# facebookresearch/GPU-DPF

Measured on AMD Instinct MI355X. Metric: DPFs/sec, higher is better.
Workload: dtype int32; 1 GPU; model=dpf-pir, entries=1048576, entry_size=16, prf=AES128, batch_per_gpu=512, global_batch=512, parallelism=dp1-replicated

## Files before the change

### csrc/hip/prf_device.h

```cpp
#pragma once
#include "hip_util.h"

namespace gpudpf_hip {

__device__ __forceinline__ uint4 add128(uint4 a, uint4 b) {
  u64 alo = ((u64)a.y << 32) | a.x, ahi = ((u64)a.w << 32) | a.z;
  u64 blo = ((u64)b.y << 32) | b.x, bhi = ((u64)b.w << 32) | b.z;
  u64 lo = alo + blo;
  u64 hi = ahi + bhi + (lo < alo ? 1u : 0u);
  return make_uint4((u32)lo, (u32)(lo >> 32), (u32)hi, (u32)(hi >> 32));
}

__device__ __forceinline__ u32 rotl(u32 v, int s) {
  return (v << s) | (v >> (32 - s));
}
__device__ __forceinline__ u32 rotr8(u32 v) { return (v >> 8) | (v << 24); }

__device__ __forceinline__ uint4 key_root(const int* key) {
  const int* rp = key + kKeyRootInt;
  return make_uint4((u32)rp[0], (u32)rp[1], (u32)rp[2], (u32)rp[3]);
}

__device__ __forceinline__ uint4 prf_dummy_full(uint4 seed, u32 pos) {
  unsigned __int128 s =
      ((unsigned __int128)(((u64)seed.w << 32) | seed.z) << 64) |
      (((u64)seed.y << 32) | seed.x);
  unsigned __int128 m = (unsigned __int128)(pos + 4242u);
  unsigned __int128 r = s * m + m;
  u64 lo = (u64)r, hi = (u64)(r >> 64);
  return make_uint4((u32)lo, (u32)(lo >> 32), (u32)hi, (u32)(hi >> 32));
}

template <int N>
__device__ __forceinline__ void stream_init(u32 (&x)[16][N], int pos_w,
                                            const u32 (&init)[16]) {
#pragma unroll
  for (int w = 0; w < 16; ++w)
#pragma unroll
    for (int i = 0; i < N; ++i) x[w][i] = init[w] + (w == pos_w ? i : 0);
}

template <int N>
__device__ __forceinline__ uint4 stream_out(const u32 (&x)[16][N], int i,
                                            int lo, uint4 seed) {
  return make_uint4(x[lo][i] + seed.x, x[lo - 1][i] + seed.y,
                    x[lo - 2][i] + seed.z, x[lo - 3][i] + seed.w);
}

template <int PART = 4, int N>
__device__ __forceinline__ void salsa_qr(u32 (&x)[16][N], int a, int b, int c,
                                         int d) {
  auto step = [&](int t, int p, int q, int s) {
#pragma unroll
    for (int i = 0; i < N; ++i) x[t][i] ^= rotl(x[p][i] + x[q][i], s);
  };
  step(b, a, d, 7);
  if constexpr (PART > 1) step(c, b, a, 9);
  if constexpr (PART > 2) step(d, c, b, 13);
  if constexpr (PART > 3) step(a, d, c, 18);
}

template <bool LOW, int N>
__device__ __forceinline__ void salsa12(uint4 seed, u32 pos, u32 (&x)[16][N]) {
  stream_init(x, 9, {0x65787061u, seed.w, seed.z, seed.y, seed.x, 0x6e642033u,
                     0, 0, 0, pos, 0x322d6279u, 0, 0, 0, 0, 0x7465206bu});
#pragma unroll
  for (int r = 0; r < (LOW ? 5 : 6); ++r) {
    salsa_qr(x, 0, 4, 8, 12);
    salsa_qr(x, 5, 9, 13, 1);
    salsa_qr(x, 10, 14, 2, 6);
    salsa_qr(x, 15, 3, 7, 11);
    salsa_qr(x, 0, 1, 2, 3);
    salsa_qr(x, 5, 6, 7, 4);
    salsa_qr(x, 10, 11, 8, 9);
    salsa_qr(x, 15, 12, 13, 14);
  }
  if constexpr (LOW) {
    salsa_qr<1>(x, 0, 4, 8, 12);
    salsa_qr(x, 5, 9, 13, 1);
    salsa_qr<3>(x, 10, 14, 2, 6);
    salsa_qr<2>(x, 15, 3, 7, 11);
    salsa_qr<3>(x, 5, 6, 7, 4);
  }
}

__device__ __forceinline__ uint4 salsa12_core(uint4 seed, u32 pos) {
  u32 x[16][1];
  salsa12<false>(seed, pos, x);
  return stream_out(x, 0, 4, seed);
}

__device__ __forceinline__ void salsa12_pair_core(uint4 seed, uint4& r0,
                                                  uint4& r1) {
  u32 x[16][2];
  salsa12<false>(seed, 0, x);
  r0 = stream_out(x, 0, 4, seed);
  r1 = stream_out(x, 1, 4, seed);
}

__device__ __forceinline__ void salsa12_pair_low_core(uint4 seed, u32& lo0,
                                                      u32& lo1) {
  u32 x[16][2];
  salsa12<true>(seed, 0, x);
  lo0 = x[4][0] + seed.x;
  lo1 = x[4][1] + seed.x;
}

template <int PART = 8, int N>
__device__ __forceinline__ void chacha_qr(u32 (&x)[16][N], int a, int b, int c,
                                          int d) {
  static_assert(PART >= 6 && PART <= 8, "only the tail is ever pruned");
  auto add = [&](int t, int s) {
#pragma unroll
    for (int i = 0; i < N; ++i) x[t][i] += x[s][i];
  };
  auto xor_rotl = [&](int t, int s, int r) {
#pragma unroll
    for (int i = 0; i < N; ++i) x[t][i] ^= x[s][i];
#pragma unroll
    for (int i = 0; i < N; ++i) x[t][i] = rotl(x[t][i], r);
  };
  add(a, b);  xor_rotl(d, a, 16);
  add(c, d);  xor_rotl(b, c, 12);
  add(a, b);  xor_rotl(d, a, 8);
  if constexpr (PART > 6) add(c, d);
  if constexpr (PART > 7) xor_rotl(b, c, 7);
}

template <bool LOW, int N>
__device__ __forceinline__ void chacha12(uint4 seed, u32 pos,
                                         u32 (&x)[16][N]) {
  stream_init(x, 13, {0x65787061u, 0x6e642033u, 0x322d6279u, 0x7465206bu,
                      seed.w, seed.z, seed.y, seed.x, 0, 0, 0, 0, 0, pos, 0, 0});
#pragma unroll
  for (int r = 0; r < (LOW ? 5 : 6); ++r) {
    chacha_qr(x, 0, 4, 8, 12);
    chacha_qr(x, 1, 5, 9, 13);
    chacha_qr(x, 2, 6, 10, 14);
    chacha_qr(x, 3, 7, 11, 15);
    chacha_qr(x, 0, 5, 10, 15);
    chacha_qr(x, 1, 6, 11, 12);
    chacha_qr(x, 2, 7, 8, 13);
    chacha_qr(x, 3, 4, 9, 14);
  }
  if constexpr (LOW) {
    chacha_qr<7>(x, 0, 4, 8, 12);
    chacha_qr<6>(x, 1, 5, 9, 13);
    chacha_qr(x, 2, 6, 10, 14);
    chacha_qr(x, 3, 7, 11, 15);
    chacha_qr(x, 2, 7, 8, 13);
  }
}

__device__ __forceinline__ uint4 chacha12_core(uint4 seed, u32 pos) {
  u32 x[16][1];
  chacha12<false>(seed, pos, x);
  return stream_out(x, 0, 7, seed);
}

__device__ __forceinline__ void chacha12_pair_core(uint4 seed, uint4& r0,
                                                   uint4& r1) {
  u32 x[16][2];
  chacha12<false>(seed, 0, x);
  r0 = stream_out(x, 0, 7, seed);
  r1 = stream_out(x, 1, 7, seed);
}

__device__ __forceinline__ void chacha12_pair_low_core(uint4 seed, u32& lo0,
                                                       u32& lo1) {
  u32 x[16][2];
  chacha12<true>(seed, 0, x);
  lo0 = x[7][0] + seed.x;
  lo1 = x[7][1] + seed.x;
}

constexpr int AES_COPIES = 32;
constexpr int AES_REP = AES_COPIES * 2;
constexpr int AES_LDS_WORDS = 256 * AES_REP;
constexpr u32 AES_TE2_BYTES = AES_COPIES * 4;

__host__ __device__ constexpr int aes_lds_u32(int prf) {
  return prf == PRF_AES128 ? AES_LDS_WORDS : 0;
}

__device__ __forceinline__ u32 xor3(u32 a, u32 b, u32 c) {
  return __builtin_amdgcn_bitop3_b32(a, b, c, 0x96);
}

template <int PA, int PB, int BA = 2, int BB = 2>
__device__ __forceinline__ u32 aes_sb_pair(u32 ta, u32 tb) {
  static_assert(PA != PB, "the two bytes land in different places");
  constexpr u32 sel = (0x0c0c0c0cu & ~(0xffu << (8 * PA)) &
                       ~(0xffu << (8 * PB))) |
                      ((4u + BA) << (8 * PA)) | ((u32)BB << (8 * PB));
  return __builtin_amdgcn_perm(ta, tb, sel);
}

__device__ __forceinline__ u32 bswap_rol8(u32 x) {
  return __builtin_amdgcn_perm(0u, x, 0x01020300u);
}

struct AesLds {
  u32 lane4;
  static __device__ __forceinline__ AesLds lane() {
    return AesLds{((u32)threadIdx.x & (u32)(AES_COPIES - 1)) << 2};
  }
  typedef __attribute__((address_space(3))) const u32 lds_u32;
  static __device__ __forceinline__ u32 ld(u32 byte_addr) {
    return *reinterpret_cast<lds_u32*>(byte_addr);
  }
  static __device__ __forceinline__ u32 ld_te2(u32 byte_addr) {
    return reinterpret_cast<lds_u32*>(byte_addr)[AES_TE2_BYTES / 4];
  }
  template <int K>
  __device__ __forceinline__ u32 addr_b(u32 w) const {
    return __builtin_amdgcn_perm(w, lane4, 0x0c0c0000u | ((4u + K) << 8));
  }
  template <int K>
  __device__ __forceinline__ u32 te0_b(u32 w) const { return ld(addr_b<K>(w)); }
  template <int K>
  __device__ __forceinline__ u32 te2_b(u32 w) const {
    return ld_te2(addr_b<K>(w));
  }
  template <int K>
  __device__ __forceinline__ u32 addr_kb(u32 q) const {
    return addr_b<(K + 1) & 3>(q);
  }
  template <int K>
  __device__ __forceinline__ u32 te0_kb(u32 q) const { return ld(addr_kb<K>(q)); }
  template <int K>
  __device__ __forceinline__ u32 te2_kb(u32 q) const {
    return ld_te2(addr_kb<K>(q));
  }
  static __device__ __forceinline__ u32 mix(u32 te0a, u32 te0b, u32 te2c,
                                            u32 te2d, u32 q) {
    return xor3(te0a, te2c, rotr8(xor3(te0b, te2d, q)));
  }
  struct Words { u32 a, b, c, d; };
  __device__ __forceinline__ Words col_issue(u32 a, u32 b, u32 c, u32 d) const {
    return {te0_b<3>(a), te0_b<2>(b), te2_b<1>(c), te2_b<0>(d)};
  }
  static __device__ __forceinline__ u32 mix(const Words& l, u32 q) {
    return mix(l.a, l.b, l.c, l.d, q);
  }
  __device__ __forceinline__ Words last_issue(u32 a, u32 b, u32 c,
                                              u32 d) const {
    return {te0_b<3>(a), te0_b<2>(b), te0_b<1>(c), te0_b<0>(d)};
  }
  static __device__ __forceinline__ u32 last(const Words& l, u32 q) {
    return xor3(aes_sb_pair<0, 3>(l.a, l.b), aes_sb_pair<2, 1>(l.c, l.d), q);
  }
  __device__ __forceinline__ Words key_issue(u32 q3) const {
    return {te0_b<2>(q3), te0_b<1>(q3), te0_b<0>(q3), te0_b<3>(q3)};
  }
  static __device__ __forceinline__ u32 key(const Words& l, u32 q0) {
    return xor3(aes_sb_pair<3, 2>(l.a, l.b), aes_sb_pair<1, 0>(l.c, l.d), q0);
  }
};

template <int PRF>
__device__ __forceinline__ void aes_stage_table(
    u32* lds0, const u32* __restrict__ aes_tabs) {
  if constexpr (PRF == PRF_AES128) {
    for (int idx = (int)threadIdx.x; idx < AES_LDS_WORDS;
         idx += (int)blockDim.x)
      lds0[idx] = aes_tabs[(((idx >> 5) & 1) << 9) + (idx >> 6)];
  }
}

template <int PRF>
__device__ __forceinline__ AesLds aes_lds_init(
    u32* lds0, const u32* __restrict__ aes_tabs) {
  aes_stage_table<PRF>(lds0, aes_tabs);
  if constexpr (PRF == PRF_AES128) __syncthreads();
  return AesLds::lane();
}

template <bool LOW>
__device__ __forceinline__ void aes_cipher_pair(uint4 seed, const AesLds& T,
                                                uint4& ra, uint4& rb) {
  u32 q0 = bswap_rol8(seed.x), q1 = bswap_rol8(seed.y),
      q2 = bswap_rol8(seed.z), q3 = bswap_rol8(seed.w);
  u32 rcon = 0x02u;
  const u32 a0 = T.addr_kb<3>(q0);
  const u32 x03 = AesLds::ld(a0), x02 = T.te0_kb<2>(q0),
            x01 = T.te2_kb<1>(q0), x00 = T.te2_kb<0>(q0);
  const u32 x13 = T.te0_kb<3>(q1), x12 = T.te0_kb<2>(q1),
            x11 = T.te2_kb<1>(q1), x10 = T.te2_kb<0>(q1);
  const u32 x23 = T.te0_kb<3>(q2), x22 = T.te0_kb<2>(q2),
            x21 = T.te2_kb<1>(q2), x20 = T.te2_kb<0>(q2);
  const u32 x33 = T.te0_kb<3>(q3), x32 = T.te0_kb<2>(q3),
            x31 = T.te2_kb<1>(q3), x30 = T.te2_kb<0>(q3);
  const u32 x03b = AesLds::ld(a0 ^ 256u);
  __builtin_amdgcn_sched_barrier(0);
  q0 = xor3(aes_sb_pair<3, 2, 0, 0>(x31, x30), aes_sb_pair<1, 0>(x33, x32),
            q0) ^ 0x01u;
  q1 ^= q0; q2 ^= q1; q3 ^= q2;
  u32 s0 = AesLds::mix(x03, x12, x21, x30, q0);
  u32 s1 = AesLds::mix(x13, x22, x31, x00, q1);
  u32 s2 = AesLds::mix(x23, x32, x01, x10, q2);
  u32 s3 = AesLds::mix(x33, x02, x11, x20, q3);
  u32 u0 = xor3(s0, x03, x03b), u1 = s1, u2 = s2, u3 = s3;
  using Words = AesLds::Words;
  u32 q[4] = {q0, q1, q2, q3};
  Words kw = T.key_issue(q[3]);
  auto key_step = [&](bool issue_next) {
    q[0] = AesLds::key(kw, q[0]) ^ rcon;
    rcon = (rcon << 1) ^ ((rcon & 0x80u) ? 0x11bu : 0u);
    rcon &= 0xffu;
    q[1] ^= q[0]; q[2] ^= q[1]; q[3] ^= q[2];
    if (issue_next) kw = T.key_issue(q[3]);
  };
  const Words e1 = T.col_issue(s1, s1, s1, s1),
              e2 = T.col_issue(s2, s2, s2, s2),
              e3 = T.col_issue(s3, s3, s3, s3);
  auto need = [](int i, int r) { return !(LOW && r == 10 && i > 0); };
  auto issue = [&](const u32 (&x)[4], int i, int r) -> Words {
    if (r == 2) {
      switch (i) {
        case 0: return {T.te0_b<3>(x[0]), e1.b, e2.c, e3.d};
        case 1: return {e1.a, e2.b, e3.c, T.te2_b<0>(x[0])};
        case 2: return {e2.a, e3.b, T.te2_b<1>(x[0]), e1.d};
        default: return {e3.a, T.te0_b<2>(x[0]), e1.c, e2.d};
      }
    }
    const u32 a = x[i], b = x[(i + 1) & 3], c = x[(i + 2) & 3],
              d = x[(i + 3) & 3];
    return r == 10 ? T.last_issue(a, b, c, d) : T.col_issue(a, b, c, d);
  };
  Words l[2][4];
  u32 st[2][4] = {{s0, s1, s2, s3}, {u0, u1, u2, u3}}, n[2][4];
  u32 out[2][4] = {{0, 0, 0, 0}, {0, 0, 0, 0}};
#pragma unroll
  for (int k = 0; k < 72 + 8; k += 4) {
#pragma unroll
    for (int j = k - 8; j < k - 4; ++j) {
      if (j < 0) continue;
      const int c = (j >> 2) & 1, i = j & 3, r = 2 + (j >> 3);
      if ((j & 7) == 0) key_step(r < 10);
      if (!need(i, r)) continue;
      if (r == 10) {
        out[c][i] = bswap_rol8(AesLds::last(l[c][i], q[i]));
      } else {
        n[c][i] = AesLds::mix(l[c][i], q[i]);
        if (i == 3) {
#pragma unroll
          for (int w = 0; w < 4; ++w) st[c][w] = n[c][w];
        }
      }
    }
#pragma unroll
    for (int j = k; j < k + 4 && j < 72; ++j) {
      const int c = (j >> 2) & 1, i = j & 3, r = 2 + (j >> 3);
      if (need(i, r)) l[c][i] = issue(st[c], i, r);
    }
    __builtin_amdgcn_sched_barrier(0);
  }
  ra = make_uint4(out[0][0], out[0][1], out[0][2], out[0][3]);
  rb = make_uint4(out[1][0], out[1][1], out[1][2], out[1][3]);
}

template <int PRF>
__device__ __forceinline__ uint4 prf_full(uint4 seed, u32 pos,
                                          const AesLds& T) {
  if constexpr (PRF == PRF_DUMMY) return prf_dummy_full(seed, pos);
  if constexpr (PRF == PRF_SALSA20) return salsa12_core(seed, pos);
  if constexpr (PRF == PRF_CHACHA20) return chacha12_core(seed, pos);
  if constexpr (PRF == PRF_AES128) {
    uint4 a, b;
    aes_cipher_pair<false>(seed, T, a, b);
    return pos ? b : a;
  }
}

template <int PRF>
__device__ __forceinline__ void prf_pair(uint4 seed, const AesLds& T,
                                         uint4& r0, uint4& r1) {
  if constexpr (PRF == PRF_AES128) {
    aes_cipher_pair<false>(seed, T, r0, r1);
  } else if constexpr (PRF == PRF_SALSA20) {
    salsa12_pair_core(seed, r0, r1);
  } else if constexpr (PRF == PRF_CHACHA20) {
    chacha12_pair_core(seed, r0, r1);
  } else {
    r0 = prf_full<PRF>(seed, 0, T);
    r1 = prf_full<PRF>(seed, 1, T);
  }
}

template <int PRF>
__device__ __forceinline__ void prf_pair_low(uint4 seed, const AesLds& T,
                                             u32& r0, u32& r1) {
  if constexpr (PRF == PRF_DUMMY) {
    r0 = seed.x * 4242u + 4242u;
    r1 = seed.x * 4243u + 4243u;
  } else if constexpr (PRF == PRF_SALSA20) {
    salsa12_pair_low_core(seed, r0, r1);
  } else if constexpr (PRF == PRF_CHACHA20) {
    chacha12_pair_low_core(seed, r0, r1);
  } else {
    uint4 a, b;
    aes_cipher_pair<true>(seed, T, a, b);
    r0 = a.x;
    r1 = b.x;
  }
}

}
```

Before: 42290 dpfs/s.

## Fold AES round byte extraction and rotation into SDWA-xor address generation

```diff
diff --git a/csrc/hip/prf_device.h b/csrc/hip/prf_device.h
--- a/csrc/hip/prf_device.h
+++ b/csrc/hip/prf_device.h
@@ -14,7 +14,6 @@
 __device__ __forceinline__ u32 rotl(u32 v, int s) {
   return (v << s) | (v >> (32 - s));
 }
-__device__ __forceinline__ u32 rotr8(u32 v) { return (v >> 8) | (v << 24); }
 
 __device__ __forceinline__ uint4 key_root(const int* key) {
   const int* rp = key + kKeyRootInt;
@@ -178,6 +177,7 @@
 constexpr int AES_REP = AES_COPIES * 2;
 constexpr int AES_LDS_WORDS = 256 * AES_REP;
 constexpr u32 AES_TE2_BYTES = AES_COPIES * 4;
+constexpr int AES_ADDR_POOL = 2;
 
 __host__ __device__ constexpr int aes_lds_u32(int prf) {
   return prf == PRF_AES128 ? AES_LDS_WORDS : 0;
@@ -219,33 +219,35 @@
   template <int K>
   __device__ __forceinline__ u32 te0_b(u32 w) const { return ld(addr_b<K>(w)); }
   template <int K>
-  __device__ __forceinline__ u32 te2_b(u32 w) const {
-    return ld_te2(addr_b<K>(w));
-  }
-  template <int K>
   __device__ __forceinline__ u32 addr_kb(u32 q) const {
     return addr_b<(K + 1) & 3>(q);
   }
-  template <int K>
-  __device__ __forceinline__ u32 te0_kb(u32 q) const { return ld(addr_kb<K>(q)); }
-  template <int K>
-  __device__ __forceinline__ u32 te2_kb(u32 q) const {
-    return ld_te2(addr_kb<K>(q));
-  }
-  static __device__ __forceinline__ u32 mix(u32 te0a, u32 te0b, u32 te2c,
-                                            u32 te2d, u32 q) {
-    return xor3(te0a, te2c, rotr8(xor3(te0b, te2d, q)));
+  struct Halves { u32 p, r; };
+  static __device__ __forceinline__ Halves halves(u32 te0a, u32 te0b,
+                                                  u32 te2c, u32 te2d, u32 q) {
+    return {te0a ^ te2c, xor3(te0b, te2d, q)};
+  }
+  template <int K>
+  static __device__ __forceinline__ void set_addr_h(u32& addr,
+                                                    const Halves& w) {
+    asm("v_xor_b32_sdwa %0, %1, %2 dst_sel:BYTE_1 dst_unused:UNUSED_PRESERVE "
+        "src0_sel:BYTE_%3 src1_sel:BYTE_%4"
+        : "+v"(addr)
+        : "v"(w.p), "v"(w.r), "n"(K), "n"((K + 1) & 3));
+  }
+  template <int K>
+  static __device__ __forceinline__ u32 te0_h(u32& addr, const Halves& w) {
+    set_addr_h<K>(addr, w);
+    return ld(addr);
+  }
+  template <int K>
+  static __device__ __forceinline__ u32 te2_h(u32& addr, const Halves& w) {
+    set_addr_h<K>(addr, w);
+    return ld_te2(addr);
   }
   struct Words { u32 a, b, c, d; };
-  __device__ __forceinline__ Words col_issue(u32 a, u32 b, u32 c, u32 d) const {
-    return {te0_b<3>(a), te0_b<2>(b), te2_b<1>(c), te2_b<0>(d)};
-  }
-  static __device__ __forceinline__ u32 mix(const Words& l, u32 q) {
-    return mix(l.a, l.b, l.c, l.d, q);
-  }
-  __device__ __forceinline__ Words last_issue(u32 a, u32 b, u32 c,
-                                              u32 d) const {
-    return {te0_b<3>(a), te0_b<2>(b), te0_b<1>(c), te0_b<0>(d)};
+  static __device__ __forceinline__ Halves halves(const Words& l, u32 q) {
+    return halves(l.a, l.b, l.c, l.d, q);
   }
   static __device__ __forceinline__ u32 last(const Words& l, u32 q) {
     return xor3(aes_sb_pair<0, 3>(l.a, l.b), aes_sb_pair<2, 1>(l.c, l.d), q);
@@ -282,25 +284,34 @@
   u32 q0 = bswap_rol8(seed.x), q1 = bswap_rol8(seed.y),
       q2 = bswap_rol8(seed.z), q3 = bswap_rol8(seed.w);
   u32 rcon = 0x02u;
-  const u32 a0 = T.addr_kb<3>(q0);
-  const u32 x03 = AesLds::ld(a0), x02 = T.te0_kb<2>(q0),
-            x01 = T.te2_kb<1>(q0), x00 = T.te2_kb<0>(q0);
-  const u32 x13 = T.te0_kb<3>(q1), x12 = T.te0_kb<2>(q1),
-            x11 = T.te2_kb<1>(q1), x10 = T.te2_kb<0>(q1);
-  const u32 x23 = T.te0_kb<3>(q2), x22 = T.te0_kb<2>(q2),
-            x21 = T.te2_kb<1>(q2), x20 = T.te2_kb<0>(q2);
-  const u32 x33 = T.te0_kb<3>(q3), x32 = T.te0_kb<2>(q3),
-            x31 = T.te2_kb<1>(q3), x30 = T.te2_kb<0>(q3);
-  const u32 x03b = AesLds::ld(a0 ^ 256u);
+  const u32 a1[16] = {
+      T.addr_kb<3>(q0), T.addr_kb<2>(q0), T.addr_kb<1>(q0), T.addr_kb<0>(q0),
+      T.addr_kb<3>(q1), T.addr_kb<2>(q1), T.addr_kb<1>(q1), T.addr_kb<0>(q1),
+      T.addr_kb<3>(q2), T.addr_kb<2>(q2), T.addr_kb<1>(q2), T.addr_kb<0>(q2),
+      T.addr_kb<3>(q3), T.addr_kb<2>(q3), T.addr_kb<1>(q3), T.addr_kb<0>(q3)};
+  static_assert(AES_ADDR_POOL >= 1 && AES_ADDR_POOL <= 16, "seeded from a1");
+  u32 ad[AES_ADDR_POOL];
+#pragma unroll
+  for (int s = 0; s < AES_ADDR_POOL; ++s) ad[s] = a1[s];
+  const u32 x03 = AesLds::ld(a1[0]), x02 = AesLds::ld(a1[1]),
+            x01 = AesLds::ld_te2(a1[2]), x00 = AesLds::ld_te2(a1[3]);
+  const u32 x13 = AesLds::ld(a1[4]), x12 = AesLds::ld(a1[5]),
+            x11 = AesLds::ld_te2(a1[6]), x10 = AesLds::ld_te2(a1[7]);
+  const u32 x23 = AesLds::ld(a1[8]), x22 = AesLds::ld(a1[9]),
+            x21 = AesLds::ld_te2(a1[10]), x20 = AesLds::ld_te2(a1[11]);
+  const u32 x33 = AesLds::ld(a1[12]), x32 = AesLds::ld(a1[13]),
+            x31 = AesLds::ld_te2(a1[14]), x30 = AesLds::ld_te2(a1[15]);
+  const u32 x03b = AesLds::ld(a1[0] ^ 256u);
   __builtin_amdgcn_sched_barrier(0);
   q0 = xor3(aes_sb_pair<3, 2, 0, 0>(x31, x30), aes_sb_pair<1, 0>(x33, x32),
             q0) ^ 0x01u;
   q1 ^= q0; q2 ^= q1; q3 ^= q2;
-  u32 s0 = AesLds::mix(x03, x12, x21, x30, q0);
-  u32 s1 = AesLds::mix(x13, x22, x31, x00, q1);
-  u32 s2 = AesLds::mix(x23, x32, x01, x10, q2);
-  u32 s3 = AesLds::mix(x33, x02, x11, x20, q3);
-  u32 u0 = xor3(s0, x03, x03b), u1 = s1, u2 = s2, u3 = s3;
+  using Halves = AesLds::Halves;
+  const Halves h1[4] = {AesLds::halves(x03, x12, x21, x30, q0),
+                        AesLds::halves(x13, x22, x31, x00, q1),
+                        AesLds::halves(x23, x32, x01, x10, q2),
+                        AesLds::halves(x33, x02, x11, x20, q3)};
+  const Halves h1b0 = {xor3(h1[0].p, x03, x03b), h1[0].r};
   using Words = AesLds::Words;
   u32 q[4] = {q0, q1, q2, q3};
   Words kw = T.key_issue(q[3]);
@@ -311,48 +322,49 @@
     q[1] ^= q[0]; q[2] ^= q[1]; q[3] ^= q[2];
     if (issue_next) kw = T.key_issue(q[3]);
   };
-  const Words e1 = T.col_issue(s1, s1, s1, s1),
-              e2 = T.col_issue(s2, s2, s2, s2),
-              e3 = T.col_issue(s3, s3, s3, s3);
   auto need = [](int i, int r) { return !(LOW && r == 10 && i > 0); };
-  auto issue = [&](const u32 (&x)[4], int i, int r) -> Words {
-    if (r == 2) {
-      switch (i) {
-        case 0: return {T.te0_b<3>(x[0]), e1.b, e2.c, e3.d};
-        case 1: return {e1.a, e2.b, e3.c, T.te2_b<0>(x[0])};
-        case 2: return {e2.a, e3.b, T.te2_b<1>(x[0]), e1.d};
-        default: return {e3.a, T.te0_b<2>(x[0]), e1.c, e2.d};
-      }
-    }
-    const u32 a = x[i], b = x[(i + 1) & 3], c = x[(i + 2) & 3],
-              d = x[(i + 3) & 3];
-    return r == 10 ? T.last_issue(a, b, c, d) : T.col_issue(a, b, c, d);
+  auto spread = [&](Words (&nl)[4], int w, const Halves& x, int r) {
+    const int ia = w, ib = (w + 3) & 3, ic = (w + 2) & 3, id = (w + 1) & 3;
+    u32 &ad_a = ad[(4 * w + 0) % AES_ADDR_POOL],
+        &ad_b = ad[(4 * w + 1) % AES_ADDR_POOL],
+        &ad_c = ad[(4 * w + 2) % AES_ADDR_POOL],
+        &ad_d = ad[(4 * w + 3) % AES_ADDR_POOL];
+    if (need(ia, r)) nl[ia].a = AesLds::te0_h<3>(ad_a, x);
+    if (need(ib, r)) nl[ib].b = AesLds::te0_h<2>(ad_b, x);
+    if (need(ic, r))
+      nl[ic].c = r == 10 ? AesLds::te0_h<1>(ad_c, x)
+                         : AesLds::te2_h<1>(ad_c, x);
+    if (need(id, r))
+      nl[id].d = r == 10 ? AesLds::te0_h<0>(ad_d, x)
+                         : AesLds::te2_h<0>(ad_d, x);
   };
+  Words e[4] = {};
+#pragma unroll
+  for (int w = 1; w < 4; ++w) spread(e, w, h1[w], 2);
   Words l[2][4];
-  u32 st[2][4] = {{s0, s1, s2, s3}, {u0, u1, u2, u3}}, n[2][4];
   u32 out[2][4] = {{0, 0, 0, 0}, {0, 0, 0, 0}};
 #pragma unroll
-  for (int k = 0; k < 72 + 8; k += 4) {
-#pragma unroll
-    for (int j = k - 8; j < k - 4; ++j) {
-      if (j < 0) continue;
-      const int c = (j >> 2) & 1, i = j & 3, r = 2 + (j >> 3);
-      if ((j & 7) == 0) key_step(r < 10);
-      if (!need(i, r)) continue;
-      if (r == 10) {
-        out[c][i] = bswap_rol8(AesLds::last(l[c][i], q[i]));
-      } else {
-        n[c][i] = AesLds::mix(l[c][i], q[i]);
-        if (i == 3) {
-#pragma unroll
-          for (int w = 0; w < 4; ++w) st[c][w] = n[c][w];
+  for (int s = 0; s < 20; ++s) {
+    const int c = s & 1, r = 1 + (s >> 1);
+    if (c == 0 && r > 1) key_step(r < 10);
+    Words nl[4] = {};
+    if (r == 1) {
+#pragma unroll
+      for (int i = 0; i < 4; ++i) nl[i] = e[i];
+      spread(nl, 0, c ? h1b0 : h1[0], 2);
+    } else {
+#pragma unroll
+      for (int w = 0; w < 4; ++w) {
+        if (r == 10) {
+          if (need(w, r)) out[c][w] = bswap_rol8(AesLds::last(l[c][w], q[w]));
+        } else {
+          spread(nl, w, AesLds::halves(l[c][w], q[w]), r + 1);
         }
       }
     }
-#pragma unroll
-    for (int j = k; j < k + 4 && j < 72; ++j) {
-      const int c = (j >> 2) & 1, i = j & 3, r = 2 + (j >> 3);
-      if (need(i, r)) l[c][i] = issue(st[c], i, r);
+    if (r < 10) {
+#pragma unroll
+      for (int i = 0; i < 4; ++i) l[c][i] = nl[i];
     }
     __builtin_amdgcn_sched_barrier(0);
   }
```

Result: faster. 43150 dpfs/s (median of 6 runs) (+2.0%).
